# lhn0323/BEVFUSION-3D_object_detection

Measured on AMD Instinct MI355X. Metric: nuScenes frames/sec (6-cam+LiDAR BEVFusion fwd+bwd), higher is better.
Workload: dtype bf16; 1 GPU; full: BEVFusion camera+LiDAR (ResNet-50, LSS 6x256x704, hard voxelize 40k pts, sparse encoder, ConvFuser, SECOND/SECONDFPN, TransFusion head + Hungarian targets + focal/L1/gaussian-focal losses) fwd + bwd + clip + AdamW, bf16 autocast, fp32 index paths; global_batch=4, points_per_frame=40000, parallelism=independent frames per rank, execution=eager launches on 2 HIP queues (camera / BEV chain, LiDAR branch), view_transform_conv_dtype=bf16, head_fp32_conv=three bf16 products per multiply, fp32 accumulation (2^-16 relative per product), dense_weight_gradients=one grouped launch per tile shape at the end of the backward pass, backward_pass_thread=caller, trainable_params=37361053

## Files before the change

bevfusion-3d_object_detection_amd/_lib.py:

```python
import ctypes
import os

import torch

_HERE = os.path.dirname(os.path.abspath(__file__))
LIB_PATH = os.path.join(_HERE, "csrc", "libbevfusion_hip.so")

_c_int = ctypes.c_int
_c_vp = ctypes.c_void_p
_c_sz = ctypes.c_size_t

SIGNATURES = {
    "bfhip_abi_version": (_c_int, []),
    "bfhip_last_error": (ctypes.c_char_p, []),
    "bfhip_profile_enable": (None, [_c_int]),
    "bfhip_profile_read": (_c_int, [_c_int, _c_vp, _c_vp, _c_int]),
    "bfhip_bev_pool_fwd": (_c_int, [_c_vp] * 5 + [_c_int] * 7 + [_c_vp, _c_vp]),
    "bfhip_bev_pool_bwd": (_c_int, [_c_vp] * 5 + [_c_int] * 8 + [_c_vp, _c_vp]),
    "bfhip_dynamic_voxelize": (_c_int, [_c_vp, _c_vp, _c_int, _c_int, _c_vp, _c_vp, _c_vp]),
    "bfhip_hard_voxelize_workspace_bytes": (_c_sz, [_c_int, _c_int, _c_int]),
    "bfhip_hard_voxelize": (_c_int, [_c_vp, _c_int, _c_int, _c_vp, _c_vp, _c_vp, _c_vp, _c_vp,
                                     _c_int, _c_int, _c_vp, _c_sz, _c_vp, _c_vp]),
    "bfhip_bev_plan_workspace_bytes": (_c_sz, [ctypes.c_longlong, ctypes.c_longlong]),
    "bfhip_bev_plan": (_c_int, [_c_vp] * 7 + [_c_int] * 4 + [_c_vp] * 3 + [_c_vp] * 11 + [_c_int, _c_vp, _c_sz, _c_vp]),
# ... 64 lines not shown
    "bfhip_decode_boxes": (_c_int, [_c_vp] * 5 + [_c_int] * 4 + [_c_vp, _c_vp, _c_vp]),
    "bfhip_assign_cost": (_c_int, [_c_vp, _c_int, _c_vp, _c_int, _c_int, _c_int, _c_vp, _c_int, _c_vp, _c_vp] + [_c_int] * 3 +
                          [_c_vp] * 4),
    "bfhip_hungarian": (_c_int, [_c_vp, _c_vp, _c_int, _c_int, _c_int, _c_vp, _c_vp, _c_vp]),
    "bfhip_assign_targets": (_c_int, [_c_vp, _c_vp, _c_vp, _c_int, _c_vp] + [_c_int] * 5 + [_c_vp] * 7),
    "bfhip_draw_heatmap": (_c_int, [_c_vp, _c_int, _c_vp, _c_vp] + [_c_int] * 5 + [_c_vp, ctypes.c_double, _c_int, _c_vp, _c_vp]),
    "bfhip_gaussian_focal_loss_workspace_bytes": (_c_sz, [ctypes.c_longlong]),
    "bfhip_gaussian_focal_loss": (_c_int, [_c_vp, _c_vp, ctypes.c_longlong, ctypes.c_float, _c_vp, _c_vp, _c_vp, _c_sz, _c_vp]),
    "bfhip_conv2d_supported": (_c_int, [_c_int] * 10),
    "bfhip_conv2d_stat_rows": (_c_int, [_c_int] * 3),
    "bfhip_conv2d_fwd": (_c_int, [_c_vp, _c_int, _c_vp, _c_vp, _c_vp, _c_int] + [_c_int] * 11 + [_c_vp, _c_vp]),
    "bfhip_conv2d_dgrad_workspace_bytes": (_c_sz, [_c_int] * 4),
    "bfhip_conv2d_dgrad": (_c_int, [_c_vp, _c_int, _c_vp, _c_vp, _c_int] + [_c_int] * 11 + [_c_vp, _c_sz, _c_vp]),
    "bfhip_conv2d_dgrad_wt": (_c_int, [_c_vp, _c_int, _c_vp, _c_vp, _c_int, _c_vp, _c_int] + [_c_int] * 11 + [_c_vp]),
    "bfhip_conv2d_dgrad_fuses_addend": (_c_int, [_c_int] * 5),
    "bfhip_split_bf16x3": (_c_int, [_c_vp, ctypes.c_longlong, _c_int, _c_vp, _c_int, _c_vp, _c_int, _c_vp]),
    "bfhip_conv2d_wt_segment_bytes": (_c_int, []),
    "bfhip_conv2d_weight_transpose_batched": (_c_int, [_c_vp, _c_int, ctypes.c_longlong, _c_vp]),
    "bfhip_conv2d_launch_choice": (_c_int, [_c_int] * 12 + [_c_vp]),
    "bfhip_conv2d_wgrad_choice": (_c_int, [_c_int] * 10 + [_c_vp]),
    "bfhip_conv2d_wgrad_workspace_bytes": (_c_sz, [_c_int] * 7),
    "bfhip_conv2d_wgrad": (_c_int, [_c_vp, _c_int, _c_vp, _c_int, _c_vp] + [_c_int] * 11 + [_c_vp, _c_sz, _c_vp]),
    "bfhip_conv2d_wgrad_group_table_bytes": (_c_sz, [_c_int]),
    "bfhip_conv2d_wgrad_groupable": (_c_int, [_c_int] * 10),
    "bfhip_conv2d_wgrad_group_plan": (_c_int, [_c_vp, _c_int, _c_int, _c_vp, _c_sz, _c_vp]),
    "bfhip_conv2d_wgrad_group_launch": (_c_int, [_c_vp, _c_vp, _c_vp, _c_sz, _c_vp]),
    "bfhip_bn2d_fwd_partials": (_c_int, [_c_vp] * 4 + [ctypes.c_longlong, _c_int, _c_int, ctypes.c_float, ctypes.c_float, _c_int] +
                                [_c_vp] * 4 + [_c_vp, _c_int, _c_vp, _c_vp]),
    "bfhip_bn2d_fwd_partials_mask": (_c_int, [_c_vp] * 4 + [ctypes.c_longlong, _c_int, _c_int, ctypes.c_float, ctypes.c_float, _c_int] +
                                     [_c_vp] * 4 + [_c_vp, _c_int, _c_vp, _c_vp, _c_vp]),
# ... 100 lines not shown
def host_f32(values):
    arr = (ctypes.c_float * len(values))(*[float(v) for v in values])
    return arr


def require_cuda(t, name):
    if not t.is_cuda:
        raise RuntimeError("%s must be a CUDA(HIP) tensor; this build has no CPU path" % name)
    if not t.is_contiguous():
        raise RuntimeError("%s must be contiguous" % name)


OPS = dict(bev_pool_fwd=0, bev_pool_bwd=1, hard_voxelize=2, dynamic_voxelize=3, lift_splat_fwd=4, lift_splat_bwd=5,
           spconv_fwd=6, spconv_bwd=7, rulebook=8, bev_aux=9, scatter_fwd=10, scatter_bwd=11, spconv_wgrad=12, raster=13,
           spconv_wgrad_main=14, conv2d_fwd=15, conv2d_dgrad=16, conv2d_wgrad=17, bn2d_fwd=18, bn2d_bwd=19,
           conv2d_pw_fwd=20, conv2d_pw_dgrad=21)


def profile_enable(on=True):
    load().bfhip_profile_enable(int(on))


def profile_read(op, reset=True):
    s = ctypes.c_double(0.0)
    c = ctypes.c_longlong(0)
    check(load().bfhip_profile_read(OPS[op] if isinstance(op, str) else op, ctypes.byref(s), ctypes.byref(c),
                                    1 if reset else 0), "profile_read")
    return s.value, c.value
```

bevfusion-3d_object_detection_amd/bn2d.py:

```python
import os

import torch
import torch.nn.functional as F
from torch import nn

from . import _lib

FUSED_BN2D = os.environ.get("BFHIP_FUSED_BN2D", "1") == "1"
RELU_BITS = os.environ.get("BFHIP_BN2D_RELU_BITS", "1") == "1"
_DT = {torch.float32: 0, torch.bfloat16: 1}
_WS = {}


def _apply(x, residual, weight, bias, running_mean, running_var, eps, momentum, relu, partial=None, rows_dev=None):
    ext = _lib.torch_ext()
    if (ext is not None and rows_dev is None and weight.dtype == torch.float32
            and (partial is None or partial.dtype == torch.float32)):
        return ext.bn2d(x, residual, weight, bias, running_mean, running_var, eps, momentum, relu, partial, RELU_BITS)
    return _BN2dFunction.apply(x, residual, weight, bias, running_mean, running_var, eps, momentum, relu, partial, rows_dev)


_SIZES = {}


# ... 110 lines not shown
                         **kw)
        self.act = act

    def fusable(self, x):
        return (FUSED_BN2D and self.training and x.is_cuda and x.dim() == 4 and x.dtype in _DT and self.affine
                and self.track_running_stats and self.momentum is not None and x.numel() > x.shape[1]
                and x.is_contiguous(memory_format=torch.channels_last)
                and _ws_bytes(x.numel() // x.shape[1], x.shape[1], _DT[x.dtype]) > 0)

    def forward(self, x, residual=None, relu=None):
        relu = self.act if relu is None else relu
        if self.fusable(x):
            self._pending_batches += 1
            partial = getattr(x, "_bfhip_stat_partial", None)
            if partial is not None:
                partial, ptr, version = partial
                if (ptr != x.data_ptr() or version != x._version or partial.shape[2] != x.shape[1]
                        or partial.shape[0] != -(-(x.numel() // x.shape[1]) // 128)):
                    partial = None
            return _apply(x, residual, self.weight, self.bias, self.running_mean, self.running_var, self.eps, self.momentum,
                          relu, partial)
        self._flush_batches()
        out = super().forward(x)
        if residual is not None:
            out = out + residual
        return F.relu(out) if relu else out

    def extra_repr(self):
        return super().extra_repr() + (", act=ReLU" if self.act else "")


class BatchNormRows(_LazyBatchCounter, nn.BatchNorm1d):

# ... 17 lines not shown
```

bevfusion-3d_object_detection_amd/conv2d.py:

```python
import os

import torch
import torch.nn.functional as F
from torch import nn

from . import _lib

ENABLED = os.environ.get("BFHIP_CONV2D", "1") == "1"
CONV_EXT = os.environ.get("BFHIP_CONV_EXT", "1") == "1"


def _conv_ext():
    if not CONV_EXT or WGRAD_SIDE_STREAM:
        return None
    ext = _lib.torch_ext()
    if ext is None or not hasattr(ext, "conv2d"):
        return None
    ext.set_wgrad_grouped(bool(WGRAD_GROUPED))
    return ext


def _cached_wt(weight):
    cached = getattr(weight, "_bfhip_wt", None)
    if cached is not None and cached[1] == weight._version and cached[2] == weight.data_ptr():
# ... 437 lines not shown
        if ctx.has_bias and ctx.needs_input_grad[2]:
            db = gn.sum(dim=(0, 1, 2))
        return dx, dw, db, None, None, None, None


class TransposedWeights:

    def __init__(self, modules):
        import numpy as np
        self.items = []
        recs = []
        blk = 0
        seg_bytes = _lib.load().bfhip_conv2d_wt_segment_bytes()
        assert seg_bytes == 40, seg_bytes
        for m in modules:
            if not isinstance(m, Conv2d) or m.groups != 1 or not m.weight.is_cuda:
                continue
            if isinstance(m, Conv2dHipWgrad) and m.dgrad != "hip" and not m.cache_wt:
                continue
            w = m.weight
            if w.dtype not in (torch.bfloat16, torch.float32) or not w.permute(0, 2, 3, 1).is_contiguous():
                continue
            Cout, Cin, KH, KW = w.shape
            wt = torch.empty(Cin * KH * KW * Cout, dtype=torch.bfloat16, device=w.device)
            self.items.append((w, wt))
            recs.append((w.data_ptr(), wt.data_ptr(), Cout, KH * KW, Cin, 1 if w.dtype == torch.float32 else 0, blk))
            blk += -(-Cin // 32) * -(-Cout // 32) * KH * KW
        self.blocks = blk
        self.table = None
        if recs:
            dt = np.dtype([("src", "<u8"), ("dst", "<u8"), ("Cout", "<i4"), ("taps", "<i4"), ("Cin", "<i4"), ("f32", "<i4"), ("blk0", "<i8")])
# ... 114 lines not shown
        if (FORK and self.fwd == "hip" and self.dgrad == "hip" and self.bias is None and self.training and torch.is_grad_enabled()
                and x.requires_grad and x.dtype == torch.bfloat16 and x.dim() == 4 and _nhwc_view(x) is not None
                and self.hip_eligible(x)):
            s, p, d = _one(self.stride), _one(self.padding), _one(self.dilation)
            y, partial, alias = conv2d(x, self.weight, None, s, p, d, True, False, 2 if subsample == 2 else 1)
            y._bfhip_stat_partial = (partial, y.data_ptr(), y._version)
            return y, alias
        return self(x), (x if subsample == 1 else None)

    def forward_unstrided(self, x_sub):
        assert self.kernel_size == (1, 1) and _one(self.padding) == 0 and self.bias is None
        y, partial = conv2d(x_sub, self.weight, None, 1, 0, 1, torch.is_grad_enabled())
        if partial is not None:
            y._bfhip_stat_partial = (partial, y.data_ptr(), y._version)
        return y
```

bevfusion-3d_object_detection_amd/csrc/capi.hip:

```cpp
#include "common.h"

#include <mutex>
#include <vector>

namespace bfhip {
static thread_local char g_err[512] = "";
void set_error(const char *fmt, ...) {
  va_list ap;
  va_start(ap, fmt);
  vsnprintf(g_err, sizeof(g_err), fmt, ap);
  va_end(ap);
}

int device_cus() {
  static std::atomic<int> cached[kMaxDevices];
  int dev = 0, v = 0;
  if (hipGetDevice(&dev) != hipSuccess) { (void)hipGetLastError(); return 256; }
  const bool slot = dev >= 0 && dev < kMaxDevices;
  if (slot && (v = cached[dev].load(std::memory_order_relaxed)) > 0) return v;
  if (hipDeviceGetAttribute(&v, hipDeviceAttributeMultiprocessorCount, dev) != hipSuccess || v <= 0) { (void)hipGetLastError(); return 256; }
  if (slot) cached[dev].store(v, std::memory_order_relaxed);
  return v;
}

static int g_prof_on = 0;
struct Pending { hipEvent_t a, b; };
static std::vector<Pending> g_pending[BFHIP_OP_COUNT];
static double g_sum_ms[BFHIP_OP_COUNT];
static long long g_count[BFHIP_OP_COUNT];
static std::mutex g_mu;

void prof_begin(int op, hipStream_t s, ProfScope *sc) {
  sc->active = false;
  if (!g_prof_on || op < 0 || op >= BFHIP_OP_COUNT) return;
  if (op >= BFHIP_OP_CONV2D_FWD && g_prof_on < 2) return;
  if (hipEventCreate(&sc->a) != hipSuccess) return;
  if (hipEventCreate(&sc->b) != hipSuccess) { hipEventDestroy(sc->a); return; }
  hipEventRecord(sc->a, s);
  sc->active = true;
  sc->op = op;
  sc->stream = s;
}

void prof_end(ProfScope *sc) {
  if (!sc->active) return;
  hipEventRecord(sc->b, sc->stream);
  std::lock_guard<std::mutex> lk(g_mu);
  g_pending[sc->op].push_back({sc->a, sc->b});
}
}
// ... 30 lines not shown
```

bevfusion-3d_object_detection_amd/csrc/conv2d.hip:

```cpp
#include "conv_common.h"

namespace bfhip {
namespace {

template <bool TR>
__device__ __forceinline__ const bf16_t *piece_src(const bf16_t *x, const ConvGeom &g, bool row_ok, int nb, int hb, int wb,
                                                   unsigned info, const bf16_t *zsrc) {
  const int dh = info >> 24, dw = (info >> 16) & 0xff, ci = info & 0xffff;
  int ih, iw;
  bool ok = row_ok;
  if (!TR) {
    ih = hb + dh;
    iw = wb + dw;
  } else {
    const int th = hb - dh, tw = wb - dw;
    ok = ok && ((th | tw) >= 0) && (((th | tw) & g.smask) == 0);
    ih = th >> g.sshift;
    iw = tw >> g.sshift;
  }
  ok = ok && (unsigned)ih < (unsigned)g.H && (unsigned)iw < (unsigned)g.W;
  const unsigned off = (unsigned)(nb + ih * g.W + iw) * (unsigned)g.ldx + (unsigned)ci;
  return ok ? x + off : zsrc;
}

// ... 7 lines not shown
    const unsigned n = mu / hw, rem = mu - n * hw;
    const unsigned i = rem / (unsigned)Wc, j = rem - i * (unsigned)Wc;
    return (long long)((n * (unsigned)H + h0 + i * stride) * (unsigned)W + w0 + j * stride);
  }
};

struct Addend {
  const bf16_t *p;
  int sub, ld, H, W;
};

template <int WGM, int WGN, int MI, int NI, bool OUT_F32, typename RowMap = RowIdentity>
__device__ __forceinline__ void igemm_epilogue(f32x16 (&acc)[MI][NI], unsigned char *smem, int tm, long long m0, int n0,
                                               long long M, int Kout, int ldy, const float *__restrict__ bias,
                                               void *__restrict__ y, float *__restrict__ stat_partial,
                                               RowMap row_map = RowMap(), Addend add = Addend{nullptr, 0, 0, 0, 0}) {
  constexpr int NTHREADS = WGM * WGN * 64;
  constexpr int BN = WGN * NI * 32, BM = WGM * MI * 32;
  constexpr int PR = BM / 128;
  constexpr int G = WGM / PR;
  static_assert(BM % 128 == 0 && G * PR == WGM, "tile rows must be whole 128-row statistic groups");
  const int tid = threadIdx.x, lane = tid & 63, w = tid >> 6;
  const int wm = w / WGN, wn = w % WGN;
  const int l31 = lane & 31, lh = lane >> 5;
  __syncthreads();

  if (stat_partial) {
    float *sred = (float *)(smem);
#pragma unroll
    for (int ni = 0; ni < NI; ++ni) {
      float s = 0.f, s2 = 0.f;
// ... 10 lines not shown
      }
    }
    __syncthreads();
    const int total_rows = (int)((M + 127) / 128);
    for (int e = tid; e < PR * BN; e += NTHREADS) {
      const int pr = e / BN, col = e - pr * BN;
      const int prow = tm * PR + pr;
      if (n0 + col < Kout && prow < total_rows) {
        float t0 = 0.f, t1 = 0.f;
#pragma unroll
        for (int gi = 0; gi < G; ++gi) {
          const float *q = sred + ((pr * G + gi) * BN + col) * 2;
          t0 += q[0];
          t1 += q[1];
        }
        stat_partial[((size_t)prow * 2 + 0) * Kout + n0 + col] = t0;
        stat_partial[((size_t)prow * 2 + 1) * Kout + n0 + col] = t1;
      }
    }
    __syncthreads();
  }

  constexpr int ESZ = OUT_F32 ? 4 : 2;
  constexpr int ROWB = BN * ESZ;
#pragma unroll
  for (int ni = 0; ni < NI; ++ni) {
    const int col = wn * (NI * 32) + ni * 32 + l31;
    const float bv = (bias && n0 + col < Kout) ? bias[n0 + col] : 0.f;
#pragma unroll
    for (int mi = 0; mi < MI; ++mi)
#pragma unroll
      for (int r = 0; r < 16; ++r) {
// ... 227 lines not shown
      bf16x8 a[MI], b[NI];
#pragma unroll
      for (int mi = 0; mi < MI; ++mi) a[mi] = *(const bf16x8 *)(pA + mi * 32 * 128 + pos);
#pragma unroll
      for (int ni = 0; ni < NI; ++ni) b[ni] = *(const bf16x8 *)(pB + ni * 32 * 128 + pos);
#pragma unroll
      for (int mi = 0; mi < MI; ++mi)
#pragma unroll
        for (int ni = 0; ni < NI; ++ni) acc[mi][ni] = __builtin_amdgcn_mfma_f32_32x32x16_bf16(a[mi], b[ni], acc[mi][ni], 0, 0, 0);
    }
    buf = buf + 1 == STAGES ? 0 : buf + 1;
    nbuf = nbuf + 1 == STAGES ? 0 : nbuf + 1;
  }
  if (MODE == 2)
    igemm_epilogue<WGM, WGN, MI, NI, OUT_F32, RowParityClass>(acc, smem, tm, m0, n0, M, g.Kout, g.ldy, bias, y, stat_partial,
                                                              RowParityClass{pc.Hc, pc.Wc, g.OH, g.OW, pc.h0, pc.w0, g.stride});
  else
    igemm_epilogue<WGM, WGN, MI, NI, OUT_F32>(acc, smem, tm, m0, n0, M, g.Kout, g.ldy, bias, y, stat_partial);
}

template <int NI, bool OUT_F32, int DIR>
__global__ __launch_bounds__(256, 4) void conv_pw_kernel(const bf16_t *__restrict__ x, const bf16_t *__restrict__ wt,
                                                         const float *__restrict__ bias, void *__restrict__ y,
                                                         float *__restrict__ stat_partial, long long M, int C, int ldx, int Kout,
                                                         int ldw, int ldy, int tiles_m, int tiles_n, Addend add) {
  constexpr int WGN = 2, MI = 2;
  constexpr int BM = 128, BN = NI * 64;
  constexpr int A_BYTES = BM * 128;
  constexpr int NA = 4, NB = BN / 32;
  extern __shared__ __attribute__((aligned(1024))) unsigned char smem[];
  const int tid = threadIdx.x, lane = tid & 63, w = tid >> 6;
// ... 308 lines not shown
BFHIP_EXPORT int bfhip_conv2d_dgrad(const void *dy, int ldg, const void *w, void *dx, int ldx, int N, int H, int W, int Cin,
                                    int Cout, int KH, int KW, int stride, int pad, int dil, int out_f32, void *workspace,
                                    size_t workspace_bytes, void *stream_) {
  BFHIP_REQUIRE(w, "conv2d_dgrad: null pointer");
  return conv2d_dgrad_impl(dy, ldg, w, dx, ldx, N, H, W, Cin, Cout, KH, KW, stride, pad, dil, out_f32, workspace, workspace_bytes,
                           (hipStream_t)stream_);
}

BFHIP_EXPORT int bfhip_conv2d_dgrad_wt(const void *dy, int ldg, const void *wt, const void *addend, int addend_stride, void *dx,
                                       int ldx, int N, int H, int W, int Cin, int Cout, int KH, int KW, int stride, int pad, int dil,
                                       int out_f32, void *stream_) {
  return conv2d_dgrad_impl(dy, ldg, nullptr, dx, ldx, N, H, W, Cin, Cout, KH, KW, stride, pad, dil, out_f32, (void *)wt,
                           bfhip_conv2d_dgrad_workspace_bytes(Cin, Cout, KH, KW), (hipStream_t)stream_, addend, addend_stride);
}

BFHIP_EXPORT int bfhip_conv2d_dgrad_fuses_addend(int KH, int KW, int stride, int pad, int out_f32) {
  return KH == 1 && KW == 1 && stride == 1 && pad == 0 && !out_f32 ? 1 : 0;
}

BFHIP_EXPORT int bfhip_split_bf16x3(const float *src, long long P, int C, void *chan, int order_chan, void *batch, int order_batch,
                                    void *stream_) {
  BFHIP_REQUIRE(src && (chan || batch) && P > 0 && C > 0 && C % 8 == 0, "split_bf16x3: bad arguments");
  BFHIP_REQUIRE(((uintptr_t)src % 16) == 0 && ((uintptr_t)chan % 16) == 0 && ((uintptr_t)batch % 16) == 0, "split_bf16x3: misaligned tensor");
  const long long total = P * (C / 8);
  BFHIP_REQUIRE(total < (1LL << 31) * 256, "split_bf16x3: tensor too large");
  hipLaunchKernelGGL(split_bf16x3_kernel, dim3((unsigned)ceil_div(total, 256)), dim3(256), 0, (hipStream_t)stream_, src, P, C,
                     (bf16_t *)chan, order_chan, (bf16_t *)batch, order_batch);
  return check_launch("split_bf16x3");
}

// ... 9 lines not shown
```

bevfusion-3d_object_detection_amd/csrc/conv_common.h:

```cpp
#pragma once
#include "common.h"
#include <stddef.h>

namespace bfhip {
namespace {

typedef unsigned short bf16_t;
typedef __attribute__((ext_vector_type(8))) __bf16 bf16x8;
typedef __attribute__((ext_vector_type(4))) short short4_t;
typedef __attribute__((ext_vector_type(16))) float f32x16;

constexpr int kZeroLines = 1024;
__device__ __attribute__((aligned(4096))) unsigned g_zero_page[kZeroLines * 16];

__device__ __forceinline__ const unsigned short *zero_src() {
  const unsigned line = (blockIdx.x * 8u + (threadIdx.x >> 6)) & (unsigned)(kZeroLines - 1);
  return (const unsigned short *)(g_zero_page + line * 16u);
}

struct ConvGeom {
  int N, H, W, C, ldx;
  int OH, OW;
  int KH, KW, stride, pad, dil;
  int transposed;
  int sshift, smask;
  int nq;
  long long M;
  int Kout;
  int ldw;
  int ldy;
  struct ParityClass { int h0, w0, Hc, Wc, kh0, kw0, nkh, nkw, tile0; } cls[17];
  int ncls;
};

__device__ __forceinline__ unsigned rne_bf16(float f) {
  unsigned u = __float_as_uint(f);
  if ((u & 0x7fffffffu) > 0x7f800000u) return (u >> 16) | 0x40u;
  return (u + 0x7fffu + ((u >> 16) & 1u)) >> 16;
}

__device__ __forceinline__ void glds16(const void *src, void *lds_dst) {
  __builtin_amdgcn_global_load_lds((const void __attribute__((address_space(1))) *)src,
                                   (void __attribute__((address_space(3))) *)lds_dst, 16, 0, 0);
}

__device__ __forceinline__ void build_tap_table(unsigned *taps, const ConvGeom &g) {
// ... 32 lines not shown
  return g;
}

inline ConvGeom conv_geom_dgrad(int N, int H, int W, int Cin, int ldx, int Cout, int ldg, int KH, int KW, int stride, int pad,
                                int dil, bool parity) {
  ConvGeom g = {};
  g.N = N; g.H = conv_out_dim(H, KH, stride, pad, dil); g.W = conv_out_dim(W, KW, stride, pad, dil); g.C = Cout; g.ldx = ldg;
  g.OH = H; g.OW = W;
  g.KH = KH; g.KW = KW; g.stride = stride; g.pad = pad; g.dil = dil; g.transposed = 1;
  g.sshift = __builtin_ctz((unsigned)stride); g.smask = stride - 1;
  g.nq = KH * KW * Cout / 8;
  g.M = (long long)N * H * W;
  g.Kout = Cin; g.ldw = KH * KW * Cout; g.ldy = ldx;
  if (stride > 1 && stride <= 4 && dil == 1 && parity) {
    g.transposed = 2;
    for (int ph = 0; ph < stride; ++ph)
      for (int pw = 0; pw < stride; ++pw) {
        ConvGeom::ParityClass &c = g.cls[g.ncls];
        c.kh0 = ph; c.kw0 = pw;
        c.nkh = ph < KH ? (KH - ph + stride - 1) / stride : 0;
        c.nkw = pw < KW ? (KW - pw + stride - 1) / stride : 0;
        if (c.nkh == 0 || c.nkw == 0) c.nkh = c.nkw = 0;
        c.h0 = ((ph - pad) % stride + stride) % stride;
        c.w0 = ((pw - pad) % stride + stride) % stride;
        c.Hc = c.h0 < H ? (H - c.h0 + stride - 1) / stride : 0;
        c.Wc = c.w0 < W ? (W - c.w0 + stride - 1) / stride : 0;
        c.tile0 = 0;
        if (c.Hc > 0 && c.Wc > 0) ++g.ncls;
      }
  }
  return g;
}

struct SplitPlan { int splits; long long rows_per_split; };
inline SplitPlan plan_splits(long long steps, int tiles, int slots, int min_steps) {
  long long want = tiles >= slots ? 1 : slots / tiles;
  if (want > steps / min_steps) want = steps / min_steps;
  if (want < 1) want = 1;
  const long long per = (steps + want - 1) / want;
  return {(int)((steps + per - 1) / per), per * 64};
}

}
// ... 2 lines not shown
```

bevfusion-3d_object_detection_amd/csrc/torch_binding.cpp:

```cpp
#include <torch/extension.h>
#include <torch/csrc/autograd/engine.h>
#include <torch/csrc/autograd/graph_task.h>
#include <c10/hip/HIPStream.h>
#include <c10/hip/HIPGuard.h>
#include <ATen/hip/impl/HIPStreamMasqueradingAsCUDA.h>
#include <hip/hip_runtime_api.h>

#include <map>
#include <mutex>
#include <vector>

#include "../../include/bevfusion_hip.h"

namespace {

using torch::Tensor;
using torch::autograd::AutogradContext;
using torch::autograd::tensor_list;

inline void *cur_stream(const Tensor &t) { return (void *)c10::hip::getCurrentHIPStream(t.get_device()).stream(); }
inline int dt_code(const Tensor &t) { return t.scalar_type() == at::kBFloat16 ? 1 : 0; }
inline void check(int rc, const char *what) {
  TORCH_CHECK(rc == 0, what, " failed (rc=", rc, "): ", bfhip_last_error());
}
// ... 441 lines not shown
    tensor_list out(7);
    if (!grads[0].defined()) return out;
    Tensor dy = as_nhwc_bf16(grads[0]);
    if (ctx->needs_input_grad(0))
      out[0] = g[3] ? hip_dgrad(dy, x, weight, wt, stride, pad, dil, Tensor(), 1) : lib_dgrad(dy, x, weight, stride, pad, dil);
    if (ctx->needs_input_grad(1)) out[1] = launch_wgrad(x, dy, weight, stride, pad, dil);
    return out;
  }
};

Tensor lib_conv2d(const Tensor &x, const Tensor &weight, int64_t stride, int64_t pad, int64_t dil, bool dgrad_hip,
                  const c10::optional<Tensor> &wt) {
  return LibConvFn::apply(x, weight, stride, pad, dil, dgrad_hip, wt);
}

}

PYBIND11_MODULE(TORCH_EXTENSION_NAME, m) {
  m.doc() = "C++ autograd front-ends over libbevfusion_hip.so (include/bevfusion_hip.h)";
  m.def("bn2d", &bn2d, "fused BatchNorm2d(+residual)(+ReLU), channels-last, training mode; optional statistics partials of the producing conv",
        pybind11::arg("x"), pybind11::arg("residual"), pybind11::arg("weight"), pybind11::arg("bias"), pybind11::arg("running_mean"),
        pybind11::arg("running_var"), pybind11::arg("eps"), pybind11::arg("momentum"), pybind11::arg("relu"),
        pybind11::arg("partial") = c10::optional<Tensor>(), pybind11::arg("relu_bits") = false);
  m.def("bn1d", &bn1d, "fused BatchNorm1d(+residual)(+ReLU) on f32[N, C], training mode");
  m.def("conv2d", &conv2d, "dense convolution on csrc/conv2d.hip (conv2d.py::_Conv2dFunction): [y, partial (empty without statistics)[, x']]",
        pybind11::arg("x"), pybind11::arg("weight"), pybind11::arg("bias"), pybind11::arg("stride"), pybind11::arg("pad"), pybind11::arg("dil"),
        pybind11::arg("emit_stats"), pybind11::arg("dgrad_lib"), pybind11::arg("fork"), pybind11::arg("wt"));
  m.def("lib_conv2d", &lib_conv2d, "library forward, HIP weight gradient (conv2d.py::_LibConvHipWgradFunction)", pybind11::arg("x"),
        pybind11::arg("weight"), pybind11::arg("stride"), pybind11::arg("pad"), pybind11::arg("dil"), pybind11::arg("dgrad_hip"), pybind11::arg("wt"));
  m.def("defer_wgrad", &defer_wgrad, "queue a layer's weight gradient for the grouped launch at the end of the running backward pass");
  m.def("set_wgrad_grouped", [](bool on) { g_grouped = on; });
  m.def("pending_wgrads", &pending_wgrads);
  m.def("abi_version", []() { return bfhip_abi_version(); });
}
```

bevfusion-3d_object_detection_amd/dense_modules.py:

```python
import os

import torch
import torch.nn.functional as F
from torch import nn

from . import _lib
from .bn2d import BatchNorm2dAct, BatchNormRows, bn_act
from .conv2d import Conv2d, Conv2dHipWgrad, fp32_island
from .linear_rows import linear_rows
from . import attention as split_attention
from .registry import MODELS


_RESNET_CONV = os.environ.get("BFHIP_RESNET_CONV", "tuned")


def _resnet_conv(cin, cout, k, stride=1, padding=0, bias=False):
    mode = _RESNET_CONV
    if mode == "tuned":
        m = Conv2dHipWgrad(cin, cout, k, stride=stride, padding=padding, bias=bias)
        if stride == 1 and k == 1:
            m.fwd = m.dgrad = "hip"
        elif k == 3:
            m.dgrad = "hip"
# ... 253 lines not shown
            outs.append(x)
        return tuple(outs)


@MODELS.register_module()
class SECONDFPN(nn.Module):
    def __init__(self, in_channels=[128, 128, 256], out_channels=[256, 256, 256], upsample_strides=[1, 2, 4],
                 norm_cfg=dict(type="BN", eps=1e-3, momentum=0.01), upsample_cfg=dict(type="deconv", bias=False),
                 conv_cfg=dict(type="Conv2d", bias=False), use_conv_for_no_stride=False):
        super().__init__()
        eps, mom = norm_cfg.get("eps", 1e-5), norm_cfg.get("momentum", 0.1)
        deblocks = []
        for i, oc in enumerate(out_channels):
            s = upsample_strides[i]
            if s > 1 or (s == 1 and not use_conv_for_no_stride):
                up = nn.ConvTranspose2d(in_channels[i], oc, s, stride=s, bias=False)
            else:
                k = int(round(1 / s))
                up = Conv2d(in_channels[i], oc, k, stride=k, bias=False)
            deblocks.append(nn.Sequential(up, *bn_act(oc, eps=eps, momentum=mom)))
        self.deblocks = nn.ModuleList(deblocks)

    def forward(self, x):
        ups = [d(x[i]) for i, d in enumerate(self.deblocks)]
        return [torch.cat(ups, dim=1) if len(ups) > 1 else ups[0]]


class PositionEncodingLearned(nn.Module):

    def __init__(self, input_channel, num_pos_feats=288):
        super().__init__()
# ... 323 lines not shown
```

include/bevfusion_hip.h:

```cpp
#ifndef BEVFUSION_HIP_H_
#define BEVFUSION_HIP_H_

#include <stddef.h>
#include <stdint.h>

#ifdef __cplusplus
extern "C" {
#endif

#define BFHIP_OK 0
#define BFHIP_E_INVALID (-1)
#define BFHIP_E_WORKSPACE (-2)
#define BFHIP_E_LAUNCH (-3)

#define BFHIP_REDUCE_SUM 0
#define BFHIP_REDUCE_MEAN 1
#define BFHIP_REDUCE_MAX 2

#define BFHIP_OP_BEV_POOL_FWD 0
#define BFHIP_OP_BEV_POOL_BWD 1
#define BFHIP_OP_HARD_VOXELIZE 2
#define BFHIP_OP_DYNAMIC_VOXELIZE 3
#define BFHIP_OP_LIFT_SPLAT_FWD 4
#define BFHIP_OP_LIFT_SPLAT_BWD 5
// ... 1 lines not shown
#define BFHIP_OP_SPCONV_BWD 7
#define BFHIP_OP_RULEBOOK 8
#define BFHIP_OP_BEV_AUX 9
#define BFHIP_OP_SCATTER_FWD 10
#define BFHIP_OP_SCATTER_BWD 11
#define BFHIP_OP_SPCONV_WGRAD 12
#define BFHIP_OP_RASTER 13
#define BFHIP_OP_SPCONV_WGRAD_MAIN 14
#define BFHIP_OP_CONV2D_FWD 15
#define BFHIP_OP_CONV2D_DGRAD 16
#define BFHIP_OP_CONV2D_WGRAD 17
#define BFHIP_OP_BN2D_FWD 18
#define BFHIP_OP_BN2D_BWD 19
#define BFHIP_OP_CONV2D_PW_FWD 20
#define BFHIP_OP_CONV2D_PW_DGRAD 21
#define BFHIP_OP_COUNT 24

int bfhip_abi_version(void);
const char *bfhip_last_error(void);

void bfhip_profile_enable(int on);
int bfhip_profile_read(int op, double *sum_ms_host, long long *count_host, int reset);

int bfhip_bev_pool_fwd(const float *x, const int32_t *geom, const int32_t *starts,
                       const int32_t *lengths, float *out, int n, int c, int m, int b, int d,
                       int h, int w, const int32_t *m_dev, void *stream);
int bfhip_bev_pool_bwd(const float *out_grad, const int32_t *geom, const int32_t *starts,
                       const int32_t *lengths, float *x_grad, int n, int c, int m, int b, int d,
                       int h, int w, int intervals_cover_all_rows, const int32_t *m_dev,
                       void *stream);
// ... 174 lines not shown
int bfhip_voxel_compact_mean(const float *voxels, const int32_t *coors, const int32_t *num_points, const int32_t *counts_dev,
                             int B, int max_voxels, int P, int F, int cap, float *feats, int32_t *out_coords,
                             int32_t *n_total_dev, void *stream);

int bfhip_conv2d_supported(int N, int H, int W, int Cin, int Cout, int KH, int KW, int stride, int pad, int dil);
int bfhip_conv2d_stat_rows(int N, int OH, int OW);
int bfhip_conv2d_fwd(const void *x, int ldx, const void *w, const float *bias, void *y, int ldy, int N, int H, int W, int Cin,
                     int Cout, int KH, int KW, int stride, int pad, int dil, int out_f32, float *stat_partial, void *stream);
size_t bfhip_conv2d_dgrad_workspace_bytes(int Cin, int Cout, int KH, int KW);
int bfhip_conv2d_dgrad(const void *dy, int ldg, const void *w, void *dx, int ldx, int N, int H, int W, int Cin, int Cout,
                       int KH, int KW, int stride, int pad, int dil, int out_f32, void *workspace, size_t workspace_bytes,
                       void *stream);
int bfhip_conv2d_dgrad_wt(const void *dy, int ldg, const void *wt, const void *addend, int addend_stride, void *dx, int ldx, int N,
                          int H, int W, int Cin, int Cout, int KH, int KW, int stride, int pad, int dil, int out_f32, void *stream);
int bfhip_conv2d_dgrad_fuses_addend(int KH, int KW, int stride, int pad, int out_f32);
int bfhip_conv2d_wt_segment_bytes(void);
int bfhip_conv2d_weight_transpose_batched(const void *segs_dev, int nseg, long long total_blocks, void *stream);
int bfhip_split_bf16x3(const float *src, long long P, int C, void *chan, int order_chan, void *batch, int order_batch, void *stream);
int bfhip_conv2d_launch_choice(int dir, int N, int H, int W, int Cin, int Cout, int KH, int KW, int stride, int pad, int dil,
                               int out_f32, int32_t *out_host);
int bfhip_conv2d_wgrad_choice(int N, int H, int W, int Cin, int Cout, int KH, int KW, int stride, int pad, int dil,
                              int32_t *out_host);
size_t bfhip_conv2d_wgrad_workspace_bytes(int N, int OH, int OW, int Cin, int Cout, int KH, int KW);
int bfhip_conv2d_wgrad(const void *x, int ldx, const void *dy, int ldg, void *dw, int N, int H, int W, int Cin, int Cout,
                       int KH, int KW, int stride, int pad, int dil, int dw_bf16, void *workspace, size_t workspace_bytes,
                       void *stream);
typedef struct bfhip_wgrad_layer {
  const void *x, *dy;
  void *dw;
  int32_t ldx, ldg, N, H, W, Cin, Cout, KH, KW, stride, pad, dil, dw_bf16, reserved;
// ... 46 lines not shown
```

Before: 155.7 frames/s.

## Route SECONDFPN transposed convs through HIP parity-class igemm with fused BN stats

Replaces nn.ConvTranspose2d (kernel equals stride) in the SECONDFPN neck with a custom HIP path. The forward reuses the strided-dgrad parity-class implicit GEMM and emits BatchNorm partial statistics from its epilogue, using per-class stat row offsets. The backward uses the conv2d forward kernel for the data gradient and the HIP wgrad for the weight gradient. The aim is to avoid the library deconvolution and a separate BN statistics pass, at the cost of more custom code and a new stat-row layout that BN has to recognise.

```diff
diff --git a/bevfusion-3d_object_detection_amd/_lib.py b/bevfusion-3d_object_detection_amd/_lib.py
--- a/bevfusion-3d_object_detection_amd/_lib.py
+++ b/bevfusion-3d_object_detection_amd/_lib.py
@@ -102,6 +102,9 @@
     "bfhip_conv2d_dgrad": (_c_int, [_c_vp, _c_int, _c_vp, _c_vp, _c_int] + [_c_int] * 11 + [_c_vp, _c_sz, _c_vp]),
     "bfhip_conv2d_dgrad_wt": (_c_int, [_c_vp, _c_int, _c_vp, _c_vp, _c_int, _c_vp, _c_int] + [_c_int] * 11 + [_c_vp]),
     "bfhip_conv2d_dgrad_fuses_addend": (_c_int, [_c_int] * 5),
+    "bfhip_deconv2d_supported": (_c_int, [_c_int] * 10),
+    "bfhip_deconv2d_stat_rows": (_c_int, [_c_int] * 4),
+    "bfhip_deconv2d_fwd": (_c_int, [_c_vp, _c_int, _c_vp, _c_vp, _c_int] + [_c_int] * 7 + [_c_vp, _c_vp]),
     "bfhip_split_bf16x3": (_c_int, [_c_vp, ctypes.c_longlong, _c_int, _c_vp, _c_int, _c_vp, _c_int, _c_vp]),
     "bfhip_conv2d_wt_segment_bytes": (_c_int, []),
     "bfhip_conv2d_weight_transpose_batched": (_c_int, [_c_vp, _c_int, ctypes.c_longlong, _c_vp]),
@@ -232,7 +235,7 @@
 OPS = dict(bev_pool_fwd=0, bev_pool_bwd=1, hard_voxelize=2, dynamic_voxelize=3, lift_splat_fwd=4, lift_splat_bwd=5,
            spconv_fwd=6, spconv_bwd=7, rulebook=8, bev_aux=9, scatter_fwd=10, scatter_bwd=11, spconv_wgrad=12, raster=13,
            spconv_wgrad_main=14, conv2d_fwd=15, conv2d_dgrad=16, conv2d_wgrad=17, bn2d_fwd=18, bn2d_bwd=19,
-           conv2d_pw_fwd=20, conv2d_pw_dgrad=21)
+           conv2d_pw_fwd=20, conv2d_pw_dgrad=21, deconv2d_fwd=22)
 
 
 def profile_enable(on=True):
diff --git a/bevfusion-3d_object_detection_amd/bn2d.py b/bevfusion-3d_object_detection_amd/bn2d.py
--- a/bevfusion-3d_object_detection_amd/bn2d.py
+++ b/bevfusion-3d_object_detection_amd/bn2d.py
@@ -148,9 +148,9 @@
             self._pending_batches += 1
             partial = getattr(x, "_bfhip_stat_partial", None)
             if partial is not None:
-                partial, ptr, version = partial
+                partial, ptr, version, *rows = partial
                 if (ptr != x.data_ptr() or version != x._version or partial.shape[2] != x.shape[1]
-                        or partial.shape[0] != -(-(x.numel() // x.shape[1]) // 128)):
+                        or partial.shape[0] != (rows[0] if rows else -(-(x.numel() // x.shape[1]) // 128))):
                     partial = None
             return _apply(x, residual, self.weight, self.bias, self.running_mean, self.running_var, self.eps, self.momentum,
                           relu, partial)
diff --git a/bevfusion-3d_object_detection_amd/conv2d.py b/bevfusion-3d_object_detection_amd/conv2d.py
--- a/bevfusion-3d_object_detection_amd/conv2d.py
+++ b/bevfusion-3d_object_detection_amd/conv2d.py
@@ -475,7 +475,7 @@
         seg_bytes = _lib.load().bfhip_conv2d_wt_segment_bytes()
         assert seg_bytes == 40, seg_bytes
         for m in modules:
-            if not isinstance(m, Conv2d) or m.groups != 1 or not m.weight.is_cuda:
+            if not isinstance(m, (Conv2d, ConvTranspose2dHip)) or m.groups != 1 or not m.weight.is_cuda:
                 continue
             if isinstance(m, Conv2dHipWgrad) and m.dgrad != "hip" and not m.cache_wt:
                 continue
@@ -620,3 +620,88 @@
         if partial is not None:
             y._bfhip_stat_partial = (partial, y.data_ptr(), y._version)
         return y
+
+
+DECONV = os.environ.get("BFHIP_DECONV", "hip") != "lib"
+
+
+def _deconv_wt(weight):
+    wt = _cached_wt(weight)
+    if wt is None:
+        w = weight.detach()
+        wt = (w if w.dtype == torch.bfloat16 else w.to(torch.bfloat16)).permute(1, 2, 3, 0).contiguous()
+    return wt
+
+
+class _Deconv2dFunction(torch.autograd.Function):
+    @staticmethod
+    def forward(ctx, x, weight, k, emit_stats, wt):
+        ctx.set_materialize_grads(False)
+        x = _as_nhwc_bf16(x)
+        N, Cin, H, W = x.shape
+        Cout = weight.shape[1]
+        y = torch.empty((N, H * k, W * k, Cout), dtype=torch.bfloat16, device=x.device).permute(0, 3, 1, 2)
+        partial = None
+        if emit_stats:
+            partial = torch.empty((_lib.load().bfhip_deconv2d_stat_rows(N, H, W, k), 2, Cout), dtype=torch.float32, device=x.device)
+        _lib.call("bfhip_deconv2d_fwd", x.data_ptr(), _nhwc_view(x), wt.data_ptr(), y.data_ptr(), Cout, N, H, W, Cin, Cout, k, 0,
+                  _lib.ptr(partial), _lib.stream_of(x))
+        ctx.save_for_backward(x, weight)
+        ctx.k = k
+        if partial is not None:
+            ctx.mark_non_differentiable(partial)
+        return y, partial
+
+    @staticmethod
+    def backward(ctx, dy, _dpartial):
+        x, weight = ctx.saved_tensors
+        if dy is None:
+            return None, None, None, None, None
+        k = ctx.k
+        N, Cin, H, W = x.shape
+        Cout = weight.shape[1]
+        dy = _as_nhwc_bf16(dy)
+        dx = dw = None
+        if ctx.needs_input_grad[0]:
+            dx = torch.empty((N, H, W, Cin), dtype=torch.bfloat16, device=x.device).permute(0, 3, 1, 2)
+            _lib.call("bfhip_conv2d_fwd", dy.data_ptr(), _nhwc_view(dy), _weight_ohwi(weight).data_ptr(), None, dx.data_ptr(), Cin, N,
+                      H * k, W * k, Cout, Cin, k, k, k, 0, 1, 0, None, _lib.stream_of(x))
+        if ctx.needs_input_grad[1]:
+            dw, _ = _launch_wgrad(dy, x, weight, k, 0, 1)
+        return dx, dw, None, None, None
+
+
+def deconv2d(x, weight, k, emit_stats=False):
+    wt = _deconv_wt(weight)
+    ext = _conv_ext() if x.is_cuda and x.dim() == 4 and not weight._backward_hooks else None
+    if ext is not None and hasattr(ext, "deconv2d"):
+        out = ext.deconv2d(x, weight, int(k), bool(emit_stats), wt)
+        return out[0], (out[1] if emit_stats else None)
+    return _Deconv2dFunction.apply(x, weight, int(k), bool(emit_stats), wt)
+
+
+class ConvTranspose2dHip(nn.ConvTranspose2d):
+
+    def hip_eligible(self, x):
+        if not (ENABLED and DECONV and x.is_cuda and x.dim() == 4 and self.groups == 1 and self.bias is None
+                and self.padding_mode == "zeros" and _one(self.output_padding) == 0):
+            return False
+        low = x.dtype == torch.bfloat16 or (torch.is_autocast_enabled("cuda") and torch.get_autocast_dtype("cuda") == torch.bfloat16
+                                            and x.dtype == torch.float32)
+        if not low or self.weight.dtype not in (torch.bfloat16, torch.float32) or not x.is_contiguous(memory_format=torch.channels_last):
+            return False
+        s, p, d = _one(self.stride), _one(self.padding), _one(self.dilation)
+        if s is None or p is None or d is None:
+            return False
+        N, Cin, H, W = x.shape
+        return bool(_lib.load().bfhip_deconv2d_supported(N, H, W, Cin, self.out_channels, self.kernel_size[0], self.kernel_size[1],
+                                                         s, p, d))
+
+    def forward(self, x, output_size=None):
+        if output_size is not None or not self.hip_eligible(x):
+            return super().forward(x, output_size)
+        emit = self.training and torch.is_grad_enabled()
+        y, partial = deconv2d(x, self.weight, self.kernel_size[0], emit)
+        if partial is not None:
+            y._bfhip_stat_partial = (partial, y.data_ptr(), y._version, partial.shape[0])
+        return y
diff --git a/bevfusion-3d_object_detection_amd/csrc/capi.hip b/bevfusion-3d_object_detection_amd/csrc/capi.hip
--- a/bevfusion-3d_object_detection_amd/csrc/capi.hip
+++ b/bevfusion-3d_object_detection_amd/csrc/capi.hip
@@ -33,7 +33,7 @@
 void prof_begin(int op, hipStream_t s, ProfScope *sc) {
   sc->active = false;
   if (!g_prof_on || op < 0 || op >= BFHIP_OP_COUNT) return;
-  if (op >= BFHIP_OP_CONV2D_FWD && g_prof_on < 2) return;
+  if (op >= BFHIP_OP_CONV2D_FWD && op != BFHIP_OP_DECONV2D_FWD && g_prof_on < 2) return;
   if (hipEventCreate(&sc->a) != hipSuccess) return;
   if (hipEventCreate(&sc->b) != hipSuccess) { hipEventDestroy(sc->a); return; }
   hipEventRecord(sc->a, s);
diff --git a/bevfusion-3d_object_detection_amd/csrc/conv2d.hip b/bevfusion-3d_object_detection_amd/csrc/conv2d.hip
--- a/bevfusion-3d_object_detection_amd/csrc/conv2d.hip
+++ b/bevfusion-3d_object_detection_amd/csrc/conv2d.hip
@@ -45,7 +45,8 @@
 __device__ __forceinline__ void igemm_epilogue(f32x16 (&acc)[MI][NI], unsigned char *smem, int tm, long long m0, int n0,
                                                long long M, int Kout, int ldy, const float *__restrict__ bias,
                                                void *__restrict__ y, float *__restrict__ stat_partial,
-                                               RowMap row_map = RowMap(), Addend add = Addend{nullptr, 0, 0, 0, 0}) {
+                                               RowMap row_map = RowMap(), Addend add = Addend{nullptr, 0, 0, 0, 0},
+                                               int stat_row0 = 0) {
   constexpr int NTHREADS = WGM * WGN * 64;
   constexpr int BN = WGN * NI * 32, BM = WGM * MI * 32;
   constexpr int PR = BM / 128;
@@ -86,8 +87,8 @@
           t0 += q[0];
           t1 += q[1];
         }
-        stat_partial[((size_t)prow * 2 + 0) * Kout + n0 + col] = t0;
-        stat_partial[((size_t)prow * 2 + 1) * Kout + n0 + col] = t1;
+        stat_partial[((size_t)(stat_row0 + prow) * 2 + 0) * Kout + n0 + col] = t0;
+        stat_partial[((size_t)(stat_row0 + prow) * 2 + 1) * Kout + n0 + col] = t1;
       }
     }
     __syncthreads();
@@ -345,7 +346,8 @@
   }
   if (MODE == 2)
     igemm_epilogue<WGM, WGN, MI, NI, OUT_F32, RowParityClass>(acc, smem, tm, m0, n0, M, g.Kout, g.ldy, bias, y, stat_partial,
-                                                              RowParityClass{pc.Hc, pc.Wc, g.OH, g.OW, pc.h0, pc.w0, g.stride});
+                                                              RowParityClass{pc.Hc, pc.Wc, g.OH, g.OW, pc.h0, pc.w0, g.stride},
+                                                              Addend{nullptr, 0, 0, 0, 0}, pc.srow0);
   else
     igemm_epilogue<WGM, WGN, MI, NI, OUT_F32>(acc, smem, tm, m0, n0, M, g.Kout, g.ldy, bias, y, stat_partial);
 }
@@ -684,6 +686,38 @@
                            bfhip_conv2d_dgrad_workspace_bytes(Cin, Cout, KH, KW), (hipStream_t)stream_, addend, addend_stride);
 }
 
+static bool deconv_ok(int N, int H, int W, int Cin, int Cout, int KH, int KW, int stride, int pad, int dil) {
+  if (KH != KW || KH != stride || (stride != 2 && stride != 4) || pad != 0 || dil != 1) return false;
+  if (N <= 0 || H <= 0 || W <= 0 || (long long)H * stride > 0x7fffffffLL / stride || (long long)W * stride > 0x7fffffffLL / stride) return false;
+  return geom_ok(N, H * stride, W * stride, Cin, KH, KW, stride, 0, 1) && geom_ok(N, H * stride, W * stride, Cout, KH, KW, stride, 0, 1) &&
+         (long long)N * H * W * stride * stride < (1LL << 31);
+}
+
+BFHIP_EXPORT int bfhip_deconv2d_supported(int N, int H, int W, int Cin, int Cout, int KH, int KW, int stride, int pad, int dil) {
+  return deconv_ok(N, H, W, Cin, Cout, KH, KW, stride, pad, dil) ? 1 : 0;
+}
+
+BFHIP_EXPORT int bfhip_deconv2d_stat_rows(int N, int H, int W, int k) {
+  if ((k != 2 && k != 4) || N <= 0 || H <= 0 || W <= 0) return 0;
+  return k * k * ceil_div((long long)N * H * W, 128);
+}
+
+BFHIP_EXPORT int bfhip_deconv2d_fwd(const void *x, int ldx, const void *wt, void *y, int ldy, int N, int H, int W, int Cin, int Cout,
+                                    int k, int out_f32, float *stat_partial, void *stream_) {
+  BFHIP_REQUIRE(deconv_ok(N, H, W, Cin, Cout, k, k, k, 0, 1), "deconv2d_fwd: unsupported geometry");
+  BFHIP_REQUIRE(x && wt && y, "deconv2d_fwd: null pointer");
+  BFHIP_REQUIRE(dma_operand_ok(x, ldx, Cin) && ((uintptr_t)wt % 16) == 0 && ldy >= Cout, kOperandMsg, "deconv2d_fwd");
+  BFHIP_REQUIRE((long long)N * H * W * ldx < (1LL << 31) && (long long)N * H * W * k * k * ldy < (1LL << 31),
+                "deconv2d_fwd: tensors of 2^31 elements or more are not supported");
+  const ConvGeom g = conv_geom_dgrad(N, H * k, W * k, Cout, ldy, Cin, ldx, k, k, k, 0, 1, true);
+  BFHIP_REQUIRE(g.transposed == 2 && g.ncls == k * k && g.H == H && g.W == W, "deconv2d_fwd: geometry");
+  ProfScope ps;
+  prof_begin(BFHIP_OP_DECONV2D_FWD, (hipStream_t)stream_, &ps);
+  const int rc = launch_igemm(x, wt, nullptr, y, stat_partial, g, out_f32, (hipStream_t)stream_, "deconv2d_fwd");
+  prof_end(&ps);
+  return rc;
+}
+
 BFHIP_EXPORT int bfhip_conv2d_dgrad_fuses_addend(int KH, int KW, int stride, int pad, int out_f32) {
   return KH == 1 && KW == 1 && stride == 1 && pad == 0 && !out_f32 ? 1 : 0;
 }
diff --git a/bevfusion-3d_object_detection_amd/csrc/conv_common.h b/bevfusion-3d_object_detection_amd/csrc/conv_common.h
--- a/bevfusion-3d_object_detection_amd/csrc/conv_common.h
+++ b/bevfusion-3d_object_detection_amd/csrc/conv_common.h
@@ -29,7 +29,7 @@
   int Kout;
   int ldw;
   int ldy;
-  struct ParityClass { int h0, w0, Hc, Wc, kh0, kw0, nkh, nkw, tile0; } cls[17];
+  struct ParityClass { int h0, w0, Hc, Wc, kh0, kw0, nkh, nkw, tile0, srow0; } cls[17];
   int ncls;
 };
 
@@ -92,6 +92,7 @@
   g.Kout = Cin; g.ldw = KH * KW * Cout; g.ldy = ldx;
   if (stride > 1 && stride <= 4 && dil == 1 && parity) {
     g.transposed = 2;
+    int srow = 0;
     for (int ph = 0; ph < stride; ++ph)
       for (int pw = 0; pw < stride; ++pw) {
         ConvGeom::ParityClass &c = g.cls[g.ncls];
@@ -104,7 +105,11 @@
         c.Hc = c.h0 < H ? (H - c.h0 + stride - 1) / stride : 0;
         c.Wc = c.w0 < W ? (W - c.w0 + stride - 1) / stride : 0;
         c.tile0 = 0;
-        if (c.Hc > 0 && c.Wc > 0) ++g.ncls;
+        c.srow0 = srow;
+        if (c.Hc > 0 && c.Wc > 0) {
+          ++g.ncls;
+          srow += (int)(((long long)N * c.Hc * c.Wc + 127) / 128);
+        }
       }
   }
   return g;
diff --git a/bevfusion-3d_object_detection_amd/csrc/torch_binding.cpp b/bevfusion-3d_object_detection_amd/csrc/torch_binding.cpp
--- a/bevfusion-3d_object_detection_amd/csrc/torch_binding.cpp
+++ b/bevfusion-3d_object_detection_amd/csrc/torch_binding.cpp
@@ -479,6 +479,49 @@
   return LibConvFn::apply(x, weight, stride, pad, dil, dgrad_hip, wt);
 }
 
+class DeconvFn : public torch::autograd::Function<DeconvFn> {
+ public:
+  static tensor_list forward(AutogradContext *ctx, const Tensor &x_, const Tensor &weight, int64_t k, bool emit_stats, const Tensor &wt) {
+    ctx->set_materialize_grads(false);
+    Tensor x = as_nhwc_bf16(x_);
+    const int64_t N = x.size(0), Cin = x.size(1), H = x.size(2), W = x.size(3), Cout = weight.size(1);
+    Tensor y = empty_nhwc(N, Cout, H * k, W * k, x.options());
+    Tensor partial = emit_stats ? at::empty({(int64_t)bfhip_deconv2d_stat_rows((int)N, (int)H, (int)W, (int)k), 2, Cout}, x.options().dtype(at::kFloat))
+                                : at::empty({0}, x.options().dtype(at::kFloat));
+    check(bfhip_deconv2d_fwd(x.data_ptr(), (int)nhwc_pitch(x), wt.data_ptr(), y.data_ptr(), (int)Cout, (int)N, (int)H, (int)W, (int)Cin,
+                             (int)Cout, (int)k, 0, emit_stats ? partial.data_ptr<float>() : nullptr, cur_stream(x)),
+          "deconv2d_fwd");
+    ctx->save_for_backward({x, weight});
+    ctx->saved_data["k"] = k;
+    ctx->mark_non_differentiable({partial});
+    return {y, partial};
+  }
+
+  static tensor_list backward(AutogradContext *ctx, tensor_list grads) {
+    auto saved = ctx->get_saved_variables();
+    const Tensor &x = saved[0], &weight = saved[1];
+    const int64_t k = ctx->saved_data["k"].toInt();
+    tensor_list out(5);
+    if (!grads[0].defined()) return out;
+    Tensor dy = as_nhwc_bf16(grads[0]);
+    const int64_t N = x.size(0), Cin = x.size(1), H = x.size(2), W = x.size(3), Cout = weight.size(1);
+    if (ctx->needs_input_grad(0)) {
+      Tensor dx = empty_nhwc(N, Cin, H, W, x.options());
+      Tensor w = weight_ohwi(weight);
+      check(bfhip_conv2d_fwd(dy.data_ptr(), (int)nhwc_pitch(dy), w.data_ptr(), nullptr, dx.data_ptr(), (int)Cin, (int)N, (int)(H * k),
+                             (int)(W * k), (int)Cout, (int)Cin, (int)k, (int)k, (int)k, 0, 1, 0, nullptr, cur_stream(x)),
+            "conv2d_fwd (deconv2d data gradient)");
+      out[0] = dx;
+    }
+    if (ctx->needs_input_grad(1)) out[1] = launch_wgrad(dy, x, weight, k, 0, 1);
+    return out;
+  }
+};
+
+tensor_list deconv2d(const Tensor &x, const Tensor &weight, int64_t k, bool emit_stats, const Tensor &wt) {
+  return DeconvFn::apply(x, weight, k, emit_stats, wt);
+}
+
 }
 
 PYBIND11_MODULE(TORCH_EXTENSION_NAME, m) {
@@ -493,6 +536,8 @@
         pybind11::arg("emit_stats"), pybind11::arg("dgrad_lib"), pybind11::arg("fork"), pybind11::arg("wt"));
   m.def("lib_conv2d", &lib_conv2d, "library forward, HIP weight gradient (conv2d.py::_LibConvHipWgradFunction)", pybind11::arg("x"),
         pybind11::arg("weight"), pybind11::arg("stride"), pybind11::arg("pad"), pybind11::arg("dil"), pybind11::arg("dgrad_hip"), pybind11::arg("wt"));
+  m.def("deconv2d", &deconv2d, "transposed convolution, kernel = stride (conv2d.py::_Deconv2dFunction): [y, partial (empty without statistics)]",
+        pybind11::arg("x"), pybind11::arg("weight"), pybind11::arg("k"), pybind11::arg("emit_stats"), pybind11::arg("wt"));
   m.def("defer_wgrad", &defer_wgrad, "queue a layer's weight gradient for the grouped launch at the end of the running backward pass");
   m.def("set_wgrad_grouped", [](bool on) { g_grouped = on; });
   m.def("pending_wgrads", &pending_wgrads);
diff --git a/bevfusion-3d_object_detection_amd/dense_modules.py b/bevfusion-3d_object_detection_amd/dense_modules.py
--- a/bevfusion-3d_object_detection_amd/dense_modules.py
+++ b/bevfusion-3d_object_detection_amd/dense_modules.py
@@ -6,7 +6,7 @@
 
 from . import _lib
 from .bn2d import BatchNorm2dAct, BatchNormRows, bn_act
-from .conv2d import Conv2d, Conv2dHipWgrad, fp32_island
+from .conv2d import Conv2d, Conv2dHipWgrad, ConvTranspose2dHip, fp32_island
 from .linear_rows import linear_rows
 from . import attention as split_attention
 from .registry import MODELS
@@ -291,7 +291,7 @@
         for i, oc in enumerate(out_channels):
             s = upsample_strides[i]
             if s > 1 or (s == 1 and not use_conv_for_no_stride):
-                up = nn.ConvTranspose2d(in_channels[i], oc, s, stride=s, bias=False)
+                up = ConvTranspose2dHip(in_channels[i], oc, s, stride=s, bias=False)
             else:
                 k = int(round(1 / s))
                 up = Conv2d(in_channels[i], oc, k, stride=k, bias=False)
diff --git a/include/bevfusion_hip.h b/include/bevfusion_hip.h
--- a/include/bevfusion_hip.h
+++ b/include/bevfusion_hip.h
@@ -39,6 +39,7 @@
 #define BFHIP_OP_BN2D_BWD 19
 #define BFHIP_OP_CONV2D_PW_FWD 20
 #define BFHIP_OP_CONV2D_PW_DGRAD 21
+#define BFHIP_OP_DECONV2D_FWD 22
 #define BFHIP_OP_COUNT 24
 
 int bfhip_abi_version(void);
@@ -243,6 +244,10 @@
 int bfhip_conv2d_dgrad_wt(const void *dy, int ldg, const void *wt, const void *addend, int addend_stride, void *dx, int ldx, int N,
                           int H, int W, int Cin, int Cout, int KH, int KW, int stride, int pad, int dil, int out_f32, void *stream);
 int bfhip_conv2d_dgrad_fuses_addend(int KH, int KW, int stride, int pad, int out_f32);
+int bfhip_deconv2d_supported(int N, int H, int W, int Cin, int Cout, int KH, int KW, int stride, int pad, int dil);
+int bfhip_deconv2d_stat_rows(int N, int H, int W, int k);
+int bfhip_deconv2d_fwd(const void *x, int ldx, const void *wt, void *y, int ldy, int N, int H, int W, int Cin, int Cout, int k,
+                       int out_f32, float *stat_partial, void *stream);
 int bfhip_conv2d_wt_segment_bytes(void);
 int bfhip_conv2d_weight_transpose_batched(const void *segs_dev, int nseg, long long total_blocks, void *stream);
 int bfhip_split_bf16x3(const float *src, long long P, int C, void *chan, int order_chan, void *batch, int order_batch, void *stream);
```

Result: no change. 156.5 frames/s (median of 6 runs) (+0.6%).
